# wwyuan2023/VITS

Hardware: AMD Instinct MI355X
Metric: 22.05 kHz audio samples/sec/GPU (infer RTF) + train utt/sec at 1/2/4/8 MI355X (higher is better)
Workload: dtype fp32; 1 GPU; SynthesizerTrn.infer_p2 batch=16 Tx=100 Ty=500 (configs/base.json, 16 kHz, hop 192) per GPU; global_batch=16, seq_len=500, parallelism=single GPU, graph=False

## Files before the change

### include/vits_amd.h

```cpp
#ifndef VITS_AMD_H
#define VITS_AMD_H

#include <stdint.h>

#ifdef __cplusplus
extern "C" {
#endif

#define VITS_OK 0
#define VITS_E_ARG (-1)
#define VITS_E_SHAPE (-2)
#define VITS_E_UNSUP (-3)


#define VITS_EPI_STORE 0
#define VITS_EPI_GATE 1
#define VITS_EPI_UPSAMPLE 2

#define VITS_ACT_NONE 0
#define VITS_ACT_RELU 1
#define VITS_ACT_TANH 2
#define VITS_ACT_EXP 3

#define VITS_TILE_128x128 0
// ... 280 lines not shown
  const float* w1;
  int32_t m_pad1;
  int32_t cin_pad1;
  int32_t kc1;
  int32_t k;
  int32_t dil;
  int32_t kc2;
  const float* b1;
  const float* cond;
  int64_t cond_bstride;
  const float* w2;
  int32_t m_pad2;
  int32_t cin_pad2;
  const float* b2;
  float* y;
  int64_t y_bstride;
  int32_t y_cstride;
  int32_t accumulate;
  float post_div;
  int32_t len_skip;
  const int32_t* lengths;
} vits_resblock_pair_desc;
int vits_resblock_pair_forward(const vits_resblock_pair_desc* d, int n, int batch, void* stream);
int vits_resblock_pair_kc(int channels, int k, int dil, int* kc1, int* kc2);
int vits_resblock_pair16_forward(const vits_resblock_pair_desc* d, int n, int batch, int wdtype,
                                 void* stream);
int vits_resblock_pair16_mean_forward(const vits_resblock_pair_desc* d, int n, int batch,
                                      int wdtype, void* stream);
int vits_resblock_pair_f32p_forward(const vits_resblock_pair_desc* d, int n, int batch,
                                    void* stream);
int vits_resblock_pair_f32p_mean_forward(const vits_resblock_pair_desc* d, int n, int batch,
                                         void* stream);

#define VITS_RADAM_MAX 96
typedef struct vits_radam_tensor {
  float* param;
  const float* grad;
  float* exp_avg;
  float* exp_avg_sq;
  int64_t numel;
} vits_radam_tensor;
int vits_radam_step(const vits_radam_tensor* tensors, int n, float* scal, const float* found_inf,
                    const float* grad_scale, double lr, const double* lr_dev, double beta1,
                    double beta2, double eps, double weight_decay, void* stream);

#define VITS_WNORM_MAX 56
typedef struct vits_wnorm_layer {
  const float* v;
  const float* g;
  float* w;
  const float* dw;
  float* dv;
  float* dg;
  int32_t rows;
  int32_t cols;
} vits_wnorm_layer;
int vits_weight_norm_forward(const vits_wnorm_layer* layers, int n, float* norms, void* stream);
int vits_weight_norm_backward(const vits_wnorm_layer* layers, int n, const float* norms,
                              void* stream);

#define VITS_SNORM_MAX 48
typedef struct vits_snorm_layer {
  const float* w;
  float* u;
  float* v;
  float* w_sn;
// ... 100 lines not shown
```

### vits_amd/_lib.py

```python
from __future__ import annotations

import ctypes as C
import os
import threading

_LIB_PATH = os.path.join(os.path.dirname(os.path.abspath(__file__)), "lib", "libvits_amd.so")
_LIB_PATH = os.environ.get("VITS_AMD_LIB", _LIB_PATH)
_lock = threading.Lock()
_lib = None

VITS_OK = 0
VITS_E_ARG = -1
VITS_E_SHAPE = -2
VITS_E_UNSUP = -3

EPI_STORE, EPI_GATE, EPI_UPSAMPLE = 0, 1, 2
ACT_NONE, ACT_RELU, ACT_TANH, ACT_EXP = 0, 1, 2, 3
TILE_128x128, TILE_64x256, TILE_32x256, TILE_64x128 = 0, 1, 2, 3
WDT_F32, WDT_BF16, WDT_F16, WDT_F32S, WDT_F32P = 0, 1, 2, 3, 4
TILE_ROWS = {TILE_128x128: 128, TILE_64x256: 64, TILE_32x256: 32, TILE_64x128: 64}
DT_F32, DT_F16, DT_BF16, DT_I32 = 0, 1, 2, 3


class ConvOut(C.Structure):
# ... 53 lines not shown

class ResblockPairDesc(C.Structure):
    _fields_ = [
        ("x", C.c_void_p),
        ("x_bstride", C.c_int64),
        ("x_cstride", C.c_int32),
        ("t_len", C.c_int32),
        ("channels", C.c_int32),
        ("in_slope", C.c_float),
        ("w1", C.c_void_p),
        ("m_pad1", C.c_int32),
        ("cin_pad1", C.c_int32),
        ("kc1", C.c_int32),
        ("k", C.c_int32),
        ("dil", C.c_int32),
        ("kc2", C.c_int32),
        ("b1", C.c_void_p),
        ("cond", C.c_void_p),
        ("cond_bstride", C.c_int64),
        ("w2", C.c_void_p),
        ("m_pad2", C.c_int32),
        ("cin_pad2", C.c_int32),
        ("b2", C.c_void_p),
        ("y", C.c_void_p),
        ("y_bstride", C.c_int64),
        ("y_cstride", C.c_int32),
        ("accumulate", C.c_int32),
        ("post_div", C.c_float),
        ("len_skip", C.c_int32),
        ("lengths", C.c_void_p),
    ]


class StftJob(C.Structure):
    _fields_ = [
        ("x", C.c_void_p),
        ("window", C.c_void_p),
        ("grad_mag", C.c_void_p),
        ("mag", C.c_void_p),
        ("re", C.c_void_p),
        ("im", C.c_void_p),
        ("grad_x", C.c_void_p),
        ("batch", C.c_int32),
        ("length", C.c_int32),
        ("n_fft", C.c_int32),
        ("hop", C.c_int32),
        ("win", C.c_int32),
        ("pad", C.c_int32),
        ("eps", C.c_float),
        ("layout", C.c_int32),
    ]


class ConvWgradDesc(C.Structure):
    _fields_ = [
        ("dy", C.c_void_p),
        ("dy_bstride", C.c_int64),
        ("dy_cstride", C.c_int32),
        ("cout", C.c_int32),
        ("x", C.c_void_p),
        ("x_bstride", C.c_int64),
        ("x_cstride", C.c_int32),
        ("cin", C.c_int32),
        ("tin", C.c_int32),
        ("n_out", C.c_int32),
        ("k", C.c_int32),
# ... 194 lines not shown
        C.c_int, [C.c_void_p, C.c_void_p, C.c_int, C.c_int, C.c_int, C.c_float, C.c_void_p]),
    "vits_conv1d_pack16": (
        C.c_int,
        [C.c_void_p] + [C.c_int] * 4 + [C.c_void_p] + [C.c_int] * 3
        + [C.c_void_p, C.c_int64, C.c_void_p],
    ),
    "vits_conv1d_pack16_pair": (
        C.c_int,
        [C.c_void_p] + [C.c_int] * 3 + [C.c_void_p] + [C.c_int] * 2 + [C.c_void_p]
        + [C.c_int] * 3 + [C.c_void_p],
    ),
    "vits_conv1d_pack16_pairs": (C.c_int, [C.POINTER(Pack16Layer), C.c_int, C.c_int,
                                           C.c_void_p]),
    "vits_conv1d_wgrad": (C.c_int, [C.POINTER(ConvWgradDesc), C.c_int, C.c_void_p]),
    "vits_conv1d_wgrad_workspace": (C.c_int64, [C.POINTER(ConvWgradDesc), C.c_int]),
    "vits_conv1d_wgrad_split": (C.c_int, [C.POINTER(ConvWgradDesc), C.c_int, C.c_void_p,
                                          C.c_int64, C.c_void_p]),
    "vits_gate_forward": (
        C.c_int,
        [C.c_void_p, C.c_int64, C.c_int32, C.c_void_p, C.c_int64, C.c_void_p, C.c_int64, C.c_int32,
         C.c_int, C.c_int, C.c_int, C.c_void_p],
    ),
    "vits_gate_backward": (
        C.c_int,
        [C.c_void_p, C.c_int64, C.c_int32, C.c_void_p, C.c_int64, C.c_int32, C.c_void_p, C.c_int64,
         C.c_void_p, C.c_int64, C.c_int32, C.c_void_p, C.c_int, C.c_int, C.c_int, C.c_void_p],
    ),
    "vits_resblock_pair_forward": (
        C.c_int, [C.POINTER(ResblockPairDesc), C.c_int, C.c_int, C.c_void_p]),
    "vits_resblock_pair_f32p_forward": (
        C.c_int, [C.POINTER(ResblockPairDesc), C.c_int, C.c_int, C.c_void_p]),
    "vits_resblock_pair_f32p_mean_forward": (
        C.c_int, [C.POINTER(ResblockPairDesc), C.c_int, C.c_int, C.c_void_p]),
    "vits_resblock_pair_kc": (
        C.c_int, [C.c_int, C.c_int, C.c_int, C.POINTER(C.c_int), C.POINTER(C.c_int)]),
    "vits_resblock_pair16_forward": (
        C.c_int, [C.POINTER(ResblockPairDesc), C.c_int, C.c_int, C.c_int, C.c_void_p]),
    "vits_resblock_pair16_mean_forward": (
        C.c_int, [C.POINTER(ResblockPairDesc), C.c_int, C.c_int, C.c_int, C.c_void_p]),
    "vits_gate_forward_io16": (
        C.c_int,
        [C.c_void_p, C.c_int64, C.c_int32, C.c_void_p, C.c_int64, C.c_void_p, C.c_int64, C.c_int32,
         C.c_int, C.c_int, C.c_int, C.c_int, C.c_void_p],
    ),
    "vits_gate_backward_io16": (
        C.c_int,
        [C.c_void_p, C.c_int64, C.c_int32, C.c_void_p, C.c_int64, C.c_int32, C.c_void_p, C.c_int64,
         C.c_void_p, C.c_int64, C.c_int32, C.c_void_p, C.c_int, C.c_int, C.c_int, C.c_int,
         C.c_void_p],
    ),
    "vits_gate_backward_io16_multi": (
        C.c_int, [C.POINTER(GateBwdJob), C.c_int, C.c_int, C.c_int, C.c_int, C.c_void_p]),
    "vits_radam_step": (
        C.c_int,
        [C.POINTER(RadamTensor), C.c_int, C.c_void_p, C.c_void_p, C.c_void_p, C.c_double,
         C.c_void_p] + [C.c_double] * 4 + [C.c_void_p],
    ),
    "vits_weight_norm_forward": (
        C.c_int, [C.POINTER(WnormLayer), C.c_int, C.c_void_p, C.c_void_p]),
    "vits_weight_norm_backward": (
        C.c_int, [C.POINTER(WnormLayer), C.c_int, C.c_void_p, C.c_void_p]),
    "vits_spectral_norm_supported": (C.c_int, [C.c_int, C.c_int]),
    "vits_spectral_norm_forward": (
        C.c_int, [C.POINTER(SnormLayer), C.c_int, C.c_int, C.c_int, C.c_void_p]),
    "vits_spectral_norm_workspace": (C.c_int64, [C.POINTER(SnormLayer), C.c_int]),
    "vits_spectral_norm_backward": (
# ... 125 lines not shown
```

### vits_amd/csrc/conv1d.hip

```cpp
#include <cstdlib>

#include "conv1d_impl.h"

namespace {

int check_desc(const vits_conv1d_desc& d, int batch) {
  VITS_CHECK_ARG(d.x && d.w && d.out0.y);
  VITS_CHECK_ARG(batch > 0 && d.cin > 0 && d.m > 0 && d.k > 0 && d.dil > 0 && d.n_out > 0);
  VITS_CHECK_SHAPE(d.kc >= 2 && (d.kc % 2) == 0 && d.cin_pad % d.kc == 0 && d.cin_pad >= d.cin);
  VITS_CHECK_SHAPE(d.m_pad % 128 == 0 && d.m_pad >= d.m);
  VITS_CHECK_SHAPE(d.tin >= 0 && d.x_tstride >= 1);
  VITS_CHECK_SHAPE(d.x_tstride != 1 || d.x_cstride >= d.tin);
  if (d.epi == VITS_EPI_GATE) VITS_CHECK_SHAPE((d.m % 2) == 0);
  if (d.epi == VITS_EPI_UPSAMPLE)
    VITS_CHECK_SHAPE(d.up_u > 0 && d.up_u <= 64 && d.m < (1 << 14) && d.m % d.up_u == 0 &&
                     d.t_out > 0);
  if (d.epi == VITS_EPI_STORE && d.split < d.m) VITS_CHECK_ARG(d.out1.y != nullptr);
  if ((reinterpret_cast<uintptr_t>(d.w) & 15) != 0) return VITS_E_SHAPE;
  VITS_CHECK_ARG(d.wdtype == VITS_WDT_F32 || d.wdtype == VITS_WDT_BF16 ||
                 d.wdtype == VITS_WDT_F16 || d.wdtype == VITS_WDT_F32S ||
                 d.wdtype == VITS_WDT_F32P);
  if (d.wdtype == VITS_WDT_F32P) VITS_CHECK_SHAPE(d.kc == 16 || d.kc == 32);
  if (d.wdtype != VITS_WDT_F32) VITS_CHECK_SHAPE((d.kc % 16) == 0);
  if (d.gmask) VITS_CHECK_ARG(d.epi == VITS_EPI_STORE && d.split >= d.m);
// ... 44 lines not shown
  }
  if (rc == VITS_OK) vits_count(which);
  return rc;
}

int conv1d_group_or_seq(const vits_conv1d_desc* d, int n, int batch, hipStream_t s) {
  if (n > 1 && n <= vits_conv::VITS_CONV_GROUP) {
    int rc = conv1d_group(d, n, batch, s);
    if (rc != VITS_E_UNSUP) return rc;
  }
  for (int i = 0; i < n; ++i) {
    int rc = conv1d_group(d + i, 1, batch, s);
    if (rc) return rc;
  }
  return VITS_OK;
}

}

extern "C" int vits_conv1d_forward(const vits_conv1d_desc* d, int batch, void* stream) {
  if (!d) return VITS_E_ARG;
  return conv1d_group(d, 1, batch, as_stream(stream));
}

extern "C" int vits_conv1d_forward_seq(const vits_conv1d_desc* d, int n, int batch, void* stream) {
  if (!d || n < 0) return VITS_E_ARG;
  for (int i = 0; i < n; ++i) {
    int rc = conv1d_group(d + i, 1, batch, as_stream(stream));
    if (rc) return rc;
  }
  return VITS_OK;
}

extern "C" int vits_conv1d_forward_groups(const vits_conv1d_desc* d, const int32_t* sizes,
                                          int ngroups, int batch, void* stream) {
  if (!d || !sizes || ngroups < 0) return VITS_E_ARG;
  int off = 0;
  for (int i = 0; i < ngroups; ++i) {
    VITS_CHECK_ARG(sizes[i] >= 1);
    int rc = conv1d_group_or_seq(d + off, sizes[i], batch, as_stream(stream));
    if (rc) return rc;
    off += sizes[i];
  }
  return VITS_OK;
}
```

### vits_amd/engine.py

```python
from __future__ import annotations

import os

import math
from typing import Optional

import torch

from . import ops
from ._lib import ACT_EXP, ACT_NONE, ACT_RELU, EPI_GATE
from .ops import PackedConv, make_desc, make_out, pack_conv, pack_conv_transpose

_PLAN_ATTR = "_vits_amd_plan"


def _param_signature(module: torch.nn.Module):
    ver = 0
    first = None
    n = 0
    for p in module.parameters():
        ver += p._version
        if first is None:
            first = (p.data_ptr(), p.device, p.dtype)
        n += 1
# ... 33 lines not shown


class _CondStack:

    def __init__(self):
        self.w, self.b, self.n = [], [], 0

    def add(self, weight: torch.Tensor, bias: Optional[torch.Tensor]) -> int:
        off = self.n
        self.w.append(_f32(weight))
        self.b.append(_f32(bias) if bias is not None else torch.zeros(
            weight.shape[0], device=weight.device))
        self.n += weight.shape[0]
        return off

    def finish(self):
        if not self.w:
            return None, None
        return torch.cat(self.w, 0).contiguous(), torch.cat(self.b, 0).contiguous()


def _linear_eff(lin: torch.nn.Module):
    return ops.weight_norm_effective(lin), lin.bias


def _conv_eff(conv: torch.nn.Module):
    return ops.weight_norm_effective(conv), conv.bias


_GROUP_BRANCHES = True
_FUSED_PAIRS = True
MEAN_PAIRS16 = True
MEAN_PAIRS_F32P = True
ACT16 = True


class GeneratorPlan:
    def __init__(self, gen):
        self.signature = None
        dev = _device_of(gen)
        self.num_kernels = gen.num_kernels
        w, b = _conv_eff(gen.conv_pre)
        self.conv_pre = pack_conv(w, b)
        self.ups = []
        self.stages = []
        conds = _CondStack()
        for i, up in enumerate(gen.ups):
            w, b = _conv_eff(up)
            self.ups.append(pack_conv_transpose(w, b, up.stride[0], up.padding[0]))
            blocks = []
            for j in range(gen.num_kernels):
                rb = gen.resblocks[i * gen.num_kernels + j]
                pairs = []
                for c1, c2, cs in zip(rb.convs1, rb.convs2, rb.conds):
                    w1, b1 = _conv_eff(c1)
                    w2, b2 = _conv_eff(c2)
                    wc, bc = _linear_eff(cs)
                    p1 = pack_conv(w1, b1, dilation=c1.dilation[0], padding=c1.padding[0],
                                   gate=True)
                    p2 = pack_conv(w2, b2, dilation=c2.dilation[0], padding=c2.padding[0])
                    alt = None
                    if (ops.PACK_PRECISION.wdtype == ops.WDT_F32S and p1.wdtype == ops.WDT_F32
                            and p2.wdtype == ops.WDT_F32):
                        alt = (ops.to_lowp(p1, ops.WDT_F32S, min_rows=0),
                               ops.to_lowp(p2, ops.WDT_F32S, min_rows=0))
                    pairs.append((p1, p2, conds.add(wc, bc), alt))
# ... 106 lines not shown
                    and all(fused[j][p][0].wdtype == ops.WDT_F32P for j in range(nk))):
                ops.resblock_pair_launch(tuple(pair_desc(j, p, xs) for j in range(nk)), B, dev,
                                         ops.WDT_F32P, mean=True)
                continue
            if cj:
                ops.conv1d_launch_seq(grouped(c1_desc(j, p) for j in cj), B, dev)
            for j in range(nk):
                kw = dict(accumulate=j > 0, post_div=float(nk) if j == nk - 1 else 1.0)
                if fused[j][p]:
                    pair_launch([j], p, [xs], **kw)
                else:
                    ops.conv1d_launch_seq([make_desc(blocks[j][p][1], gbuf[j],
                                                     make_out(xs, res=cur[j], **kw),
                                                     lengths=lengths, io16=io16)], B, dev)


class WNPlan:
    def __init__(self, wn, conds: Optional[_CondStack]):
        self.H = wn.hidden_channels
        self.n_layers = wn.n_layers
        self.cond_off = None
        if wn.gin_channels != 0:
            wc, bc = _linear_eff(wn.cond_layer)
            self.cond_off = conds.add(wc, bc)
        self.in_layers = []
        self.res_skip = []
        for i in range(wn.n_layers):
            w, b = _conv_eff(wn.in_layers[i])
            self.in_layers.append(pack_conv(w, b, dilation=wn.in_layers[i].dilation[0],
                                            padding=wn.in_layers[i].padding[0], gate=True))
            w, b = _conv_eff(wn.res_skip_layers[i])
            self.res_skip.append(pack_conv(w, b))

    def descs(self, h: torch.Tensor, skip: torch.Tensor, abuf: torch.Tensor,
              cond: Optional[torch.Tensor], lengths: Optional[torch.Tensor]):
        H = self.H
        out = []
        for i in range(self.n_layers):
            coff = 0 if self.cond_off is None else self.cond_off + 2 * H * i
            out.append(make_desc(self.in_layers[i], h, make_out(abuf),
                                 cond=cond if self.cond_off is not None else None,
                                 cond_offset=coff))
            last = i == self.n_layers - 1
            if not last:
                out.append(make_desc(self.res_skip[i], abuf, make_out(h, res=h),
                                     out1=make_out(skip, accumulate=i > 0), split=H,
                                     lengths=lengths))
            else:
                out.append(make_desc(self.res_skip[i], abuf,
                                     make_out(skip, accumulate=i > 0), lengths=lengths))
        return out


class CouplingFlowPlan:

    def __init__(self, block):
        self.signature = None
        conds = _CondStack()
        self.layers = []
        flipped = False
        for f in block.flows_reversed:
            if f.__class__.__name__ == "Flip":
                flipped = not flipped
                continue
            assert f.mean_only, "only mean-only couplings are on the hot path"
            half = f.half_channels
            wp, bp = _conv_eff(f.pre)
            wq, bq = _conv_eff(f.post)
            if flipped:
                wp = wp.flip(1)
                wq, bq = wq.flip(0), bq.flip(0)
            self.layers.append(dict(
                half=half, flipped=flipped,
                pre=pack_conv(wp, bp), post=pack_conv(wq, bq),
                wn=WNPlan(f.enc, conds)))
        assert not flipped, "odd number of Flip modules"
        self.cond_w, self.cond_b = conds.finish()
        self.H = self.layers[0]["wn"].H if self.layers else 0

    def conds(self, g):
        if self.cond_w is None:
            return None
        return ops.linear_rows(g, self.cond_w, self.cond_b)

# ... 343 lines not shown
```

### vits_amd/ops.py

```python
from __future__ import annotations

import contextlib
import ctypes as C
import math
import threading
from dataclasses import dataclass, field
from fractions import Fraction
from typing import Optional

import numpy as np
import torch

from . import _lib
from ._lib import (ACT_NONE, WDT_BF16, WDT_F16, WDT_F32, WDT_F32P, WDT_F32S, ConvDesc, ConvOut, EPI_GATE, EPI_STORE,
                   ResblockPairDesc,
                   EPI_UPSAMPLE, TILE_128x128, TILE_32x256, TILE_64x128, TILE_64x256, TILE_ROWS,
                   check)



def _stream_ptr(device: torch.device) -> int:
    return torch.cuda.current_stream(device).cuda_stream


def require_device(*tensors: torch.Tensor):
    for t in tensors:
        if t is None:
            continue
        if t.device.type != "cuda":
            raise _lib.VitsAmdError(
                "vits_amd HIP ops need tensors on a ROCm GPU (device 'cuda'); "
                f"got {t.device}. There is no CPU path.")


def _ptr(t: Optional[torch.Tensor]) -> Optional[int]:
    return None if t is None else t.data_ptr()


_WEIGHT_CACHE: dict = {}


def set_weight_cache(cache: dict) -> dict:
    global _WEIGHT_CACHE
    prev, _WEIGHT_CACHE = _WEIGHT_CACHE, cache
    return prev


def cached_weight(module: torch.nn.Module):
# ... 395 lines not shown
        check(lib.vits_conv1d_forward_groups(arr, sizes, 1, batch, stream.cuda_stream),
              "vits_conv1d_forward_groups")
        e.record(stream)
        self.records.append((s, e, sum(conv_flops(d, batch) for d in group)))
        self.peaks.append(MFMA_PEAK_TFLOPS[group[0].wdtype])
        self.shapes.append("conv " + "+".join(
            f"m{d.m}c{d.cin}k{d.k}d{d.dil}T{d.n_out}e{d.epi}t{d.tile}" for d in group))

    def launch_pairs(self, lib, group, batch, device, wdtype=None, mean=False):
        s = torch.cuda.Event(enable_timing=True)
        e = torch.cuda.Event(enable_timing=True)
        stream = torch.cuda.current_stream(device)
        s.record(stream)
        arr = (ResblockPairDesc * len(group))(*group)
        if wdtype is None:
            check(lib.vits_resblock_pair_forward(arr, len(group), batch, stream.cuda_stream),
                  "vits_resblock_pair_forward")
        elif wdtype == WDT_F32P:
            fn = (lib.vits_resblock_pair_f32p_mean_forward if mean
                  else lib.vits_resblock_pair_f32p_forward)
            check(fn(arr, len(group), batch, stream.cuda_stream),
                  "vits_resblock_pair_f32p_forward")
        else:
            fn = lib.vits_resblock_pair16_mean_forward if mean else lib.vits_resblock_pair16_forward
            check(fn(arr, len(group), batch, int(wdtype), stream.cuda_stream),
                  "vits_resblock_pair16_forward")
        e.record(stream)
        self.records.append((s, e, sum(resblock_pair_flops(d, batch) for d in group)))
        self.peaks.append(MFMA_PEAK_TFLOPS[WDT_F32 if wdtype is None else
                                           WDT_F32S if wdtype == WDT_F32P else wdtype])
        self.shapes.append("pair " + "+".join(
            f"C{d.channels}k{d.k}d{d.dil}T{d.t_len}" for d in group))

    def summary(self):
        torch.cuda.synchronize()
        ms = [s.elapsed_time(e) for s, e, _ in self.records]
        fl = [f for _, _, f in self.records]
        min_ms = sum(f / (pk * 1e9) for f, pk in zip(fl, self.peaks))
        return dict(launches=len(ms), total_ms=float(sum(ms)), total_flops=int(sum(fl)),
                    avg_ms=float(sum(ms) / max(1, len(ms))), mfma_bound_ms=float(min_ms),
                    f32s_flops=int(sum(f for f, pk in zip(fl, self.peaks)
                                       if pk == MFMA_PEAK_TFLOPS[WDT_F32S])))

    def per_launch(self):
        torch.cuda.synchronize()
        return [(lab, s.elapsed_time(e), f)
                for lab, (s, e, f) in zip(self.shapes, self.records)]


_RB_KC = {}


RESBLOCK_PAIR_MAX_K = 7


def resblock_pair_supported(c1: PackedConv, c2: PackedConv, T: int) -> bool:
    C = c2.out_channels
    return (c1.wdtype == WDT_F32 and c2.wdtype == WDT_F32 and C in (32, 64)
            and c1.m == C and c1.cin == C and c2.cin == C // 2 and c1.k == c2.k
            and c1.k <= RESBLOCK_PAIR_MAX_K and c2.dil == 1 and T % 4 == 0
            and _resblock_kc(C, c1.k, c1.dil) is not None)


F32P_PAIR_MAX_K = {32: 11, 64: 11, 128: 11, 256: 3}


# ... 89 lines not shown
    if ConvTimer.active is not None:
        return ConvTimer.active.launch_pairs(lib, group, batch, device, wdtype, mean=mean)
    arr = (ResblockPairDesc * len(group))(*group)
    fn = lib.vits_resblock_pair16_mean_forward if mean else lib.vits_resblock_pair16_forward
    check(fn(arr, len(group), batch, int(wdtype), _stream_ptr(device)),
          "vits_resblock_pair16_forward")


def resblock_pair_flops(d: ResblockPairDesc, batch: int) -> int:
    C_, k, T = d.channels, d.k, d.t_len
    return 2 * batch * T * (C_ * C_ * k + (C_ // 2) * C_ * k)


def resblock_pair_launch(descs, batch: int, device: torch.device, wdtype: int = WDT_F32,
                         mean: bool = False):
    group = tuple(descs) if isinstance(descs, (tuple, list)) else (descs,)
    lib = _lib.load()
    if mean and wdtype != WDT_F32P:
        raise NotImplementedError("branch-mean launch: split-fp32 pairs only")
    if ConvTimer.active is not None:
        return ConvTimer.active.launch_pairs(lib, group, batch, device,
                                             wdtype=WDT_F32P if wdtype == WDT_F32P else None,
                                             mean=mean)
    arr = (ResblockPairDesc * len(group))(*group)
    if wdtype == WDT_F32P:
        fn = (lib.vits_resblock_pair_f32p_mean_forward if mean
              else lib.vits_resblock_pair_f32p_forward)
        check(fn(arr, len(group), batch, _stream_ptr(device)), "vits_resblock_pair_f32p_forward")
        return
    check(lib.vits_resblock_pair_forward(arr, len(group), batch, _stream_ptr(device)),
          "vits_resblock_pair_forward")


def conv1d_launch(desc: ConvDesc, batch: int, device: torch.device):
    lib = _lib.load()
    if ConvTimer.active is not None:
        return ConvTimer.active.launch(lib, desc, batch, device)
    check(lib.vits_conv1d_forward(C.byref(desc), batch, _stream_ptr(device)), "vits_conv1d_forward")


def conv1d_launch_seq(descs, batch: int, device: torch.device):
    lib = _lib.load()
    if ConvTimer.active is not None:
        for d in descs:
            ConvTimer.active.launch(lib, d, batch, device)
        return
    flat, sizes = [], []
    for d in descs:
        group = tuple(d) if isinstance(d, (tuple, list)) else (d,)
        flat.extend(group)
        sizes.append(len(group))
    arr = (ConvDesc * len(flat))(*flat)
    sz = (C.c_int32 * len(sizes))(*sizes)
    check(lib.vits_conv1d_forward_groups(arr, sz, len(sizes), batch, _stream_ptr(device)),
          "vits_conv1d_forward_groups")


def conv1d(x: torch.Tensor, layer: PackedConv, *, in_slope: float = 1.0, act: int = ACT_NONE,
           cond: Optional[torch.Tensor] = None, residual: Optional[torch.Tensor] = None,
           res_scale: float = 1.0, lengths: Optional[torch.Tensor] = None,
           out: Optional[torch.Tensor] = None, accumulate: bool = False,
           post_div: float = 1.0, t_out: Optional[int] = None) -> torch.Tensor:
    require_device(x, cond, residual, lengths)
    B, _, T = x.shape
    io16 = x.dtype != torch.float32
    if layer.epi == EPI_UPSAMPLE:
        T_out = T * layer.up_u if t_out is None else t_out
    else:
        T_out = T
    if out is None:
        out = torch.empty(B, layer.out_channels, T_out, device=x.device, dtype=x.dtype)
    o0 = make_out(out, act=act, res=residual, res_scale=res_scale, accumulate=accumulate,
                  post_div=post_div)
    if lengths is not None:
        lengths = lengths.to(device=x.device, dtype=torch.int32).contiguous()
    d = make_desc(layer, x, o0, in_slope=in_slope, cond=cond, lengths=lengths, t_out=T_out,
                  io16=2 if io16 else 0)
    conv1d_launch(d, B, x.device)
# ... 784 lines not shown
```

Baseline: 79.67 million output samples/s.

## Fuse WaveNet layer in-conv, gate and res/skip conv into one f32p kernel

Adds a HIP kernel that runs a whole WN layer in one launch: the dilated in-layer conv on split-bf16 MFMA, the tanh·sigmoid gate kept in LDS, and the 1x1 res/skip conv with residual and skip accumulation in the epilogue. The layer ping-pongs h between two buffers instead of writing gated activations to global memory and reading them back, which removes a global round trip and one launch per layer. The engine switches to this path when shapes match (H=256, f32p weights), and a new combined sequencer lets it sit alongside ordinary conv launches. In exchange the kernel needs a large LDS footprint and a hand-tuned schedule, and final_h has to track which buffer ends up holding h.

Measured after the change: 81.32 million output samples/s, median of 6. +2.1%, better.

```diff
diff --git a/include/vits_amd.h b/include/vits_amd.h
--- a/include/vits_amd.h
+++ b/include/vits_amd.h
@@ -336,6 +336,42 @@
 int vits_resblock_pair_f32p_mean_forward(const vits_resblock_pair_desc* d, int n, int batch,
                                          void* stream);
 
+typedef struct vits_wn_layer_desc {
+  const float* h;
+  int64_t h_bstride;
+  int32_t h_cstride;
+  int32_t t_len;
+  int32_t hidden;
+  int32_t k;
+  int32_t dil;
+  int32_t last;
+  const void* w1;
+  int32_t m_pad1;
+  int32_t cin_pad1;
+  const float* b1;
+  const float* cond;
+  int64_t cond_bstride;
+  const void* w2;
+  int32_t m_pad2;
+  int32_t cin_pad2;
+  const float* b2;
+  float* h_out;
+  int64_t ho_bstride;
+  int32_t ho_cstride;
+  int32_t accumulate;
+  float* skip;
+  int64_t skip_bstride;
+  int32_t skip_cstride;
+  int32_t len_skip;
+  int32_t ng;
+  int32_t reserved;
+  const int32_t* lengths;
+} vits_wn_layer_desc;
+int vits_wn_layers_f32p_forward(const vits_wn_layer_desc* d, int n, int batch, void* stream);
+int vits_conv1d_wn_seq_forward(const vits_conv1d_desc* convs, int nconv,
+                               const vits_wn_layer_desc* wn, int nwn, const int32_t* kinds, int n,
+                               int batch, void* stream);
+
 #define VITS_RADAM_MAX 96
 typedef struct vits_radam_tensor {
   float* param;
diff --git a/vits_amd/_lib.py b/vits_amd/_lib.py
--- a/vits_amd/_lib.py
+++ b/vits_amd/_lib.py
@@ -109,6 +109,40 @@
     ]
 
 
+class WnLayerDesc(C.Structure):
+    _fields_ = [
+        ("h", C.c_void_p),
+        ("h_bstride", C.c_int64),
+        ("h_cstride", C.c_int32),
+        ("t_len", C.c_int32),
+        ("hidden", C.c_int32),
+        ("k", C.c_int32),
+        ("dil", C.c_int32),
+        ("last", C.c_int32),
+        ("w1", C.c_void_p),
+        ("m_pad1", C.c_int32),
+        ("cin_pad1", C.c_int32),
+        ("b1", C.c_void_p),
+        ("cond", C.c_void_p),
+        ("cond_bstride", C.c_int64),
+        ("w2", C.c_void_p),
+        ("m_pad2", C.c_int32),
+        ("cin_pad2", C.c_int32),
+        ("b2", C.c_void_p),
+        ("h_out", C.c_void_p),
+        ("ho_bstride", C.c_int64),
+        ("ho_cstride", C.c_int32),
+        ("accumulate", C.c_int32),
+        ("skip", C.c_void_p),
+        ("skip_bstride", C.c_int64),
+        ("skip_cstride", C.c_int32),
+        ("len_skip", C.c_int32),
+        ("ng", C.c_int32),
+        ("reserved", C.c_int32),
+        ("lengths", C.c_void_p),
+    ]
+
+
 class StftJob(C.Structure):
     _fields_ = [
         ("x", C.c_void_p),
@@ -369,6 +403,11 @@
         C.c_int, [C.POINTER(ResblockPairDesc), C.c_int, C.c_int, C.c_void_p]),
     "vits_resblock_pair_f32p_mean_forward": (
         C.c_int, [C.POINTER(ResblockPairDesc), C.c_int, C.c_int, C.c_void_p]),
+    "vits_wn_layers_f32p_forward": (
+        C.c_int, [C.POINTER(WnLayerDesc), C.c_int, C.c_int, C.c_void_p]),
+    "vits_conv1d_wn_seq_forward": (
+        C.c_int, [C.POINTER(ConvDesc), C.c_int, C.POINTER(WnLayerDesc), C.c_int,
+                  C.POINTER(C.c_int32), C.c_int, C.c_int, C.c_void_p]),
     "vits_resblock_pair_kc": (
         C.c_int, [C.c_int, C.c_int, C.c_int, C.POINTER(C.c_int), C.POINTER(C.c_int)]),
     "vits_resblock_pair16_forward": (
diff --git a/vits_amd/csrc/conv1d.hip b/vits_amd/csrc/conv1d.hip
--- a/vits_amd/csrc/conv1d.hip
+++ b/vits_amd/csrc/conv1d.hip
@@ -100,6 +100,30 @@
   return VITS_OK;
 }
 
+int vits_wn_layer_check(const vits_wn_layer_desc& d, int batch);
+int vits_wn_layer_launch(const vits_wn_layer_desc& d, int batch, hipStream_t s);
+
+extern "C" int vits_conv1d_wn_seq_forward(const vits_conv1d_desc* convs, int nconv,
+                                          const vits_wn_layer_desc* wn, int nwn,
+                                          const int32_t* kinds, int n, int batch, void* stream) {
+  if (!kinds || n < 1 || nconv < 0 || nwn < 0 || nconv + nwn != n) return VITS_E_ARG;
+  if ((nconv > 0 && !convs) || (nwn > 0 && !wn)) return VITS_E_ARG;
+  int ic = 0, iw = 0;
+  for (int i = 0; i < n; ++i) {
+    VITS_CHECK_ARG(kinds[i] == 0 || kinds[i] == 1);
+    VITS_CHECK_ARG(kinds[i] ? iw < nwn : ic < nconv);
+    const int rc = kinds[i] ? vits_wn_layer_check(wn[iw++], batch) : check_desc(convs[ic++], batch);
+    if (rc) return rc;
+  }
+  ic = iw = 0;
+  for (int i = 0; i < n; ++i) {
+    const int rc = kinds[i] ? vits_wn_layer_launch(wn[iw++], batch, as_stream(stream))
+                            : conv1d_group(convs + ic++, 1, batch, as_stream(stream));
+    if (rc) return rc;
+  }
+  return VITS_OK;
+}
+
 extern "C" int vits_conv1d_forward_groups(const vits_conv1d_desc* d, const int32_t* sizes,
                                           int ngroups, int batch, void* stream) {
   if (!d || !sizes || ngroups < 0) return VITS_E_ARG;
diff --git a/vits_amd/csrc/wn_f32p.hip b/vits_amd/csrc/wn_f32p.hip
--- /dev/null
+++ b/vits_amd/csrc/wn_f32p.hip
@@ -0,0 +1,427 @@
+#include <type_traits>
+
+#include "conv1d_impl.h"
+
+namespace {
+
+using vits_conv::fast_sigmoid;
+using vits_conv::fast_tanh;
+using vits_conv::split3_bf16x4;
+
+typedef __bf16 bf16x8 __attribute__((ext_vector_type(8)));
+typedef __bf16 bf16x4 __attribute__((ext_vector_type(4)));
+typedef __bf16 bf16x2 __attribute__((ext_vector_type(2)));
+typedef float f32x4v __attribute__((ext_vector_type(4)));
+typedef float f32x2v __attribute__((ext_vector_type(2)));
+
+struct WnArgs {
+  vits_wn_layer_desc d;
+  int batch;
+};
+
+constexpr int WN_KC = 64;
+
+__host__ __device__ inline int wn_xcols(int NG, int k, int dil) {
+  return ((NG + (k - 1) * dil + 3 + 3) >> 2) << 2;
+}
+__host__ __device__ inline int wn_lds_bytes(int H, int NG, int k, int dil) {
+  const int xs = 2 * 3 * wn_xcols(NG, k, dil) * (WN_KC + 4);
+  const int gsz = 3 * NG * (H + 8);
+  return 4 * 4 * H + 2 * (xs > gsz ? xs : gsz) + 64;
+}
+
+__device__ __forceinline__ float wn_gate(float a, float b) {
+#pragma clang fp contract(off)
+  return fast_tanh(a) * fast_sigmoid(b);
+}
+
+template <typename T>
+__device__ __forceinline__ T wn_fresh(T v) {
+  asm volatile("" : "+v"(v));
+  return v;
+}
+
+template <typename T>
+__device__ __forceinline__ const T* wn_sbase(const T* p) {
+  uint64_t u = reinterpret_cast<uint64_t>(p);
+  asm("" : "+s"(u));
+  return (const T*)reinterpret_cast<const __attribute__((address_space(1))) T*>(u);
+}
+
+template <int H, int NG>
+__global__ __launch_bounds__(H * 4, 4) void wn_layer_f32p_kernel(const WnArgs A) {
+  typedef std::integral_constant<bool, true> edge_t;
+  typedef std::integral_constant<bool, false> interior_t;
+  constexpr int M1 = 2 * H;
+  constexpr int NT = (M1 / 32) * 64;
+  constexpr int TN = NG / 32;
+  constexpr int KC = WN_KC;
+  constexpr int KCP = KC + 4;
+  constexpr int GP = H + 8;
+  constexpr int GPL = NG * GP;
+  constexpr int S1 = H / 16, S2 = H / 16;
+  static_assert(NT == H * 4 && NT <= 1024, "threads");
+  static_assert(KC / 4 == NT / 64, "staging: one channel quad per wave");
+  static_assert(NG == 32 || NG == 64, "tile columns");
+  typedef bf16x8 av_t;
+
+  const vits_wn_layer_desc& p = A.d;
+  const int b = blockIdx.z;
+  const int Tn = p.t_len;
+  const int L = p.lengths ? min(Tn, (int)p.lengths[b]) : Tn;
+  const int n0 = blockIdx.x * NG;
+  if (n0 >= Tn) return;
+  if (p.lengths && p.len_skip > 0 && n0 >= L + p.len_skip) return;
+  const int M2 = p.last ? H : 2 * H;
+
+  extern __shared__ float smem[];
+  float* const erow = smem;
+  __bf16* const reg = reinterpret_cast<__bf16*>(smem + 4 * H);
+
+  const int tid = threadIdx.x;
+  const int lane = tid & 63;
+  const int wid = __builtin_amdgcn_readfirstlane(tid >> 6);
+  const int wm = wid * 32;
+  const int l32 = lane & 31;
+  const int lhi = lane >> 5;
+
+  const int k = p.k;
+  const int dil = p.dil;
+  const int p1 = (k - 1) * dil / 2;
+  const int tw0 = n0 - p1;
+  const int xstart = tw0 & ~1;
+  const int xcols = wn_xcols(NG, k, dil);
+  const bool interior = n0 + NG <= L;
+
+  {
+    const float* cond = p.cond ? p.cond + (int64_t)b * p.cond_bstride : nullptr;
+    for (int r = tid; r < 4 * H; r += NT) {
+      float e = 0.f;
+      if (r < M1) {
+        const int idx = (r & 1) ? H + (r >> 1) : (r >> 1);
+        if (p.b1) e = p.b1[idx];
+        if (cond) e += cond[idx];
+      } else if (p.b2 && r - M1 < M2) {
+        e = p.b2[r - M1];
+      }
+      erow[r] = e;
+    }
+  }
+
+  f32x16 acc[TN];
+#pragma unroll
+  for (int j = 0; j < TN; ++j)
+#pragma unroll
+    for (int r = 0; r < 16; ++r) acc[j][r] = 0.f;
+
+  auto mma = [&](const av_t* a, const av_t* bh, const av_t* bm, const av_t* bl) {
+#pragma unroll
+    for (int ni = 0; ni < TN; ++ni) {
+      f32x16 c = acc[ni];
+      c = __builtin_amdgcn_mfma_f32_32x32x16_bf16(a[0], bl[ni], c, 0, 0, 0);
+      c = __builtin_amdgcn_mfma_f32_32x32x16_bf16(a[2], bh[ni], c, 0, 0, 0);
+      c = __builtin_amdgcn_mfma_f32_32x32x16_bf16(a[1], bm[ni], c, 0, 0, 0);
+      c = __builtin_amdgcn_mfma_f32_32x32x16_bf16(a[0], bm[ni], c, 0, 0, 0);
+      c = __builtin_amdgcn_mfma_f32_32x32x16_bf16(a[1], bh[ni], c, 0, 0, 0);
+      c = __builtin_amdgcn_mfma_f32_32x32x16_bf16(a[0], bh[ni], c, 0, 0, 0);
+      acc[ni] = c;
+    }
+  };
+  auto loadA = [&](const __bf16* w, uint32_t al, int64_t wstep, int m_pad, int s, int total,
+                   av_t* a) {
+    const __bf16* wp = w + (int64_t)(s < total ? s : total - 1) * wstep + (int64_t)wm * 8;
+    const uint32_t av = wn_fresh(al);
+#pragma unroll
+    for (int q = 0; q < 3; ++q)
+      a[q] = *reinterpret_cast<const av_t*>(
+          reinterpret_cast<const char*>(wn_sbase(wp + (int64_t)q * m_pad * 8)) + av);
+  };
+
+  constexpr int PF = TN == 1 ? 4 : 2;
+  static_assert((KC / 16) % PF == 0 && S2 % PF == 0, "ring alignment");
+  av_t ar[PF][3];
+  av_t bh[2][TN], bm[2][TN], bl[2][TN];
+
+  const float* xb = p.h + (int64_t)b * p.h_bstride;
+  {
+    const int xsh = tw0 - xstart;
+    const int nblk = xcols >> 1;
+    const int xpl = xcols * KCP;
+    __bf16* const xbuf0 = reg;
+    __bf16* const xbuf1 = reg + 3 * xpl;
+    const int tt = xstart + 2 * lane;
+    const bool xact = lane < nblk;
+    const bool xok = xact && tt >= 0 && tt < Tn;
+    const uint32_t xoff = xok ? (uint32_t)tt * 4u : 0u;
+    f32x2v xr[4];
+    auto gload = [&](int ch) __attribute__((always_inline)) {
+      const float* base = xb + (int64_t)(ch * KC + 4 * wid) * p.h_cstride;
+      const uint32_t xo = wn_fresh(xoff);
+#pragma unroll
+      for (int i = 0; i < 4; ++i) {
+        const float* row = wn_sbase(base + (int64_t)i * p.h_cstride);
+        xr[i] = *reinterpret_cast<const f32x2v*>(reinterpret_cast<const char*>(row) + xo);
+      }
+    };
+    auto lstore = [&](__bf16* xs) __attribute__((always_inline)) {
+      const int fl = wn_fresh(lane);
+      if (fl < nblk) {
+        __bf16* xh = xs + 2 * fl * KCP + 4 * wid;
+#pragma unroll
+        for (int e = 0; e < 2; ++e) {
+          f32x4v w;
+#pragma unroll
+          for (int i = 0; i < 4; ++i) w[i] = xok ? xr[i][e] : 0.f;
+          bf16x4 h4, m4, l4;
+          split3_bf16x4(w, h4, m4, l4);
+          *reinterpret_cast<bf16x4*>(xh + e * KCP) = h4;
+          *reinterpret_cast<bf16x4*>(xh + xpl + e * KCP) = m4;
+          *reinterpret_cast<bf16x4*>(xh + 2 * xpl + e * KCP) = l4;
+        }
+      }
+    };
+    auto loadB = [&](const __bf16* xs, int j, int g, av_t* bh, av_t* bm, av_t* bl) {
+      const int P4 = xpl / 4;
+#pragma unroll
+      for (int ni = 0; ni < TN; ++ni) {
+        const bf16x4* xp = reinterpret_cast<const bf16x4*>(
+            xs + (ni * 32 + l32 + j * dil + xsh) * KCP + 16 * g + 8 * lhi);
+        bh[ni] = __builtin_shufflevector(xp[0], xp[1], 0, 1, 2, 3, 4, 5, 6, 7);
+        bm[ni] = __builtin_shufflevector(xp[P4], xp[P4 + 1], 0, 1, 2, 3, 4, 5, 6, 7);
+        bl[ni] = __builtin_shufflevector(xp[2 * P4], xp[2 * P4 + 1], 0, 1, 2, 3, 4, 5, 6, 7);
+      }
+    };
+    const __bf16* wl = reinterpret_cast<const __bf16*>(p.w1);
+    const uint32_t al = (uint32_t)((lhi * 3) * p.m_pad1 + l32) * 16u;
+    const int64_t wstep = (int64_t)16 * 3 * p.m_pad1;
+    const int total = S1 * k;
+    const int nst = (KC / 16) * k;
+#pragma unroll
+    for (int i = 0; i < PF - 1; ++i) loadA(wl, al, wstep, p.m_pad1, i, total, ar[i]);
+    gload(0);
+    lstore(xbuf0);
+    __syncthreads();
+    for (int ch = 0; ch < H / KC; ++ch) {
+      const bool more = ch + 1 < H / KC;
+      if (more) gload(ch + 1);
+      const __bf16* xs = (ch & 1) ? xbuf1 : xbuf0;
+      const int s0 = ch * nst;
+      int j = 0, g = 0;
+      auto next = [&]() {
+        if (++j == k) {
+          j = 0;
+          ++g;
+        }
+      };
+      loadB(xs, 0, 0, bh[0], bm[0], bl[0]);
+      for (int st = 0; st < nst; st += PF) {
+#pragma unroll
+        for (int u = 0; u < PF; ++u) {
+          loadA(wl, al, wstep, p.m_pad1, s0 + st + u + PF - 1, total, ar[(u + PF - 1) % PF]);
+          next();
+          if (st + u + 1 < nst) loadB(xs, j, g, bh[(u + 1) & 1], bm[(u + 1) & 1], bl[(u + 1) & 1]);
+          __builtin_amdgcn_sched_barrier(0);
+          mma(ar[u], bh[u & 1], bm[u & 1], bl[u & 1]);
+          __builtin_amdgcn_sched_barrier(0);
+        }
+      }
+      if (more) lstore((ch & 1) ? xbuf0 : xbuf1);
+      __syncthreads();
+    }
+  }
+
+  __bf16* const gs = reg;
+  {
+    const int fl = wn_fresh(lane);
+    const int l32 = fl & 31, lhi = fl >> 5;
+    f32x4v er[4];
+#pragma unroll
+    for (int g = 0; g < 4; ++g)
+      er[g] = *reinterpret_cast<const f32x4v*>(erow + wm + 4 * lhi + 8 * g);
+#pragma unroll
+    for (int ni = 0; ni < TN; ++ni) {
+      const int col = ni * 32 + l32;
+#pragma unroll
+      for (int r = 0; r < 16; r += 4) {
+        const int row = wm + 4 * lhi + 8 * (r >> 2);
+        const f32x4v e = er[r >> 2];
+        const float g0 = wn_gate(acc[ni][r] + e[0], acc[ni][r + 1] + e[1]);
+        const float g1 = wn_gate(acc[ni][r + 2] + e[2], acc[ni][r + 3] + e[3]);
+        __bf16* gp = gs + col * GP + (row >> 1);
+        const f32x4v w = {g0, g1, 0.f, 0.f};
+        bf16x4 h4, m4, l4;
+        split3_bf16x4(w, h4, m4, l4);
+        *reinterpret_cast<bf16x2*>(gp) = __builtin_shufflevector(h4, h4, 0, 1);
+        *reinterpret_cast<bf16x2*>(gp + GPL) = __builtin_shufflevector(m4, m4, 0, 1);
+        *reinterpret_cast<bf16x2*>(gp + 2 * GPL) = __builtin_shufflevector(l4, l4, 0, 1);
+      }
+#pragma unroll
+      for (int r = 0; r < 16; ++r) acc[ni][r] = 0.f;
+    }
+  }
+  __syncthreads();
+  if (wm >= M2) return;
+
+  {
+    const int fl = wn_fresh(lane);
+    const int l32 = fl & 31, lhi = fl >> 5;
+    const __bf16* wl = reinterpret_cast<const __bf16*>(p.w2);
+    const uint32_t al = (uint32_t)((lhi * 3) * p.m_pad2 + l32) * 16u;
+    const int64_t wstep = (int64_t)16 * 3 * p.m_pad2;
+    const int total = S2;
+    const __bf16* gl = gs + l32 * GP + 8 * lhi;
+    int g = 0;
+    auto loadB = [&](av_t* bh, av_t* bm, av_t* bl) {
+      const __bf16* x = gl + 16 * g;
+#pragma unroll
+      for (int ni = 0; ni < TN; ++ni) {
+        bh[ni] = *reinterpret_cast<const av_t*>(x + ni * 32 * GP);
+        bm[ni] = *reinterpret_cast<const av_t*>(x + ni * 32 * GP + GPL);
+        bl[ni] = *reinterpret_cast<const av_t*>(x + ni * 32 * GP + 2 * GPL);
+      }
+      ++g;
+    };
+#pragma unroll
+    for (int i = 0; i < PF - 1; ++i) loadA(wl, al, wstep, p.m_pad2, i, total, ar[i]);
+    loadB(bh[0], bm[0], bl[0]);
+    for (int s = 0; s < total; s += PF) {
+#pragma unroll
+      for (int u = 0; u < PF; ++u) {
+        loadA(wl, al, wstep, p.m_pad2, s + u + PF - 1, total, ar[(u + PF - 1) % PF]);
+        if (s + u + 1 < total) loadB(bh[(u + 1) & 1], bm[(u + 1) & 1], bl[(u + 1) & 1]);
+        __builtin_amdgcn_sched_barrier(0);
+        mma(ar[u], bh[u & 1], bm[u & 1], bl[u & 1]);
+        __builtin_amdgcn_sched_barrier(0);
+      }
+    }
+  }
+
+  const bool to_h = !p.last && wm < H;
+  const int yr = (p.last || wm < H) ? wm : wm - H;
+  const float* const rrow = xb + (int64_t)wm * p.h_cstride;
+  float* const yb = to_h ? p.h_out + (int64_t)b * p.ho_bstride + (int64_t)yr * p.ho_cstride
+                         : p.skip + (int64_t)b * p.skip_bstride + (int64_t)yr * p.skip_cstride;
+  const int ycs = to_h ? p.ho_cstride : p.skip_cstride;
+  const bool accum = !to_h && p.accumulate;
+  auto epilogue = [&](auto edge) __attribute__((always_inline)) {
+    const int fl = wn_fresh(lane);
+    const int l32 = fl & 31, lhi = fl >> 5;
+    f32x4v e2[4];
+#pragma unroll
+    for (int g = 0; g < 4; ++g)
+      e2[g] = *reinterpret_cast<const f32x4v*>(erow + M1 + wm + 4 * lhi + 8 * g);
+#pragma unroll
+    for (int ni = 0; ni < TN; ++ni) {
+      const int t = n0 + ni * 32 + l32;
+      const bool st = decltype(edge)::value ? t < Tn : true;
+      const int tc = st ? t : 0;
+      const uint32_t xv = (uint32_t)(4 * lhi * p.h_cstride + tc) * 4u;
+      const uint32_t yv = (uint32_t)(4 * lhi * ycs + tc) * 4u;
+      auto xat = [&](int r) __attribute__((always_inline)) -> const float& {
+        const float* row = rrow + (int64_t)((r & 3) + 8 * (r >> 2)) * p.h_cstride;
+        return *reinterpret_cast<const float*>(reinterpret_cast<const char*>(row) + xv);
+      };
+      auto yat = [&](int r) __attribute__((always_inline)) -> float& {
+        float* row = yb + (int64_t)((r & 3) + 8 * (r >> 2)) * ycs;
+        return *reinterpret_cast<float*>(reinterpret_cast<char*>(row) + yv);
+      };
+      float o[16];
+#pragma unroll
+      for (int r = 0; r < 16; ++r) o[r] = acc[ni][r] + e2[r >> 2][r & 3];
+      if (to_h) {
+        float rv[16];
+#pragma unroll
+        for (int r = 0; r < 16; ++r) rv[r] = xat(r);
+#pragma unroll
+        for (int r = 0; r < 16; ++r) o[r] = rv[r] + o[r];
+      }
+      if (accum) {
+        float yo[16];
+#pragma unroll
+        for (int r = 0; r < 16; ++r) yo[r] = yat(r);
+#pragma unroll
+        for (int r = 0; r < 16; ++r) o[r] = yo[r] + o[r];
+      }
+      if (st) {
+#pragma unroll
+        for (int r = 0; r < 16; ++r) {
+          if constexpr (decltype(edge)::value) o[r] = t < L ? o[r] : 0.f;
+          yat(r) = o[r];
+        }
+      }
+    }
+  };
+  if (interior)
+    epilogue(interior_t());
+  else
+    epilogue(edge_t());
+}
+
+int wn_pick_ng(const vits_wn_layer_desc& d, int batch) {
+  if (d.ng == 32 || d.ng == 64) return d.ng;
+  const long tiles64 = (long)((d.t_len + 63) / 64) * batch;
+  return tiles64 >= 256 ? 64 : 32;
+}
+
+template <int H, int NG>
+int wn_launch(const vits_wn_layer_desc& d, int batch, hipStream_t s) {
+  const int lds = wn_lds_bytes(H, NG, d.k, d.dil);
+  if (lds > 160 * 1024) return VITS_E_UNSUP;
+  WnArgs a;
+  a.d = d;
+  a.batch = batch;
+  hipLaunchKernelGGL((wn_layer_f32p_kernel<H, NG>), dim3((d.t_len + NG - 1) / NG, 1, batch),
+                     dim3(H * 4), lds, s, a);
+  return vits_launch_status();
+}
+
+}
+
+int vits_wn_layer_check(const vits_wn_layer_desc& d, int batch) {
+  VITS_CHECK_ARG(batch >= 1 && batch <= 65535);
+  VITS_CHECK_ARG(d.h && d.w1 && d.w2 && d.skip);
+  VITS_CHECK_ARG(d.last ? d.h_out == nullptr : d.h_out != nullptr);
+  VITS_CHECK_ARG(reinterpret_cast<const void*>(d.h_out) != reinterpret_cast<const void*>(d.h) &&
+                 reinterpret_cast<const void*>(d.skip) != reinterpret_cast<const void*>(d.h) &&
+                 reinterpret_cast<const void*>(d.skip) != reinterpret_cast<const void*>(d.h_out));
+  VITS_CHECK_ARG(d.ng == 0 || d.ng == 32 || d.ng == 64);
+  VITS_CHECK_SHAPE(d.hidden == 256);
+  VITS_CHECK_SHAPE(d.k >= 1 && d.k <= 15 && (d.k & 1) == 1 && d.dil >= 1 && d.t_len > 0);
+  VITS_CHECK_SHAPE((d.k - 1) * d.dil <= 56);
+  const int m2 = d.last ? d.hidden : 2 * d.hidden;
+  VITS_CHECK_SHAPE(d.m_pad1 >= 2 * d.hidden && d.m_pad2 >= m2 && (d.m_pad1 & 3) == 0 &&
+                   (d.m_pad2 & 3) == 0);
+  VITS_CHECK_SHAPE(d.cin_pad1 == d.hidden && d.cin_pad2 == d.hidden);
+  VITS_CHECK_SHAPE((d.t_len & 3) == 0 && (d.h_cstride & 3) == 0 && (d.h_bstride & 3) == 0 &&
+                   d.h_cstride >= d.t_len && d.skip_cstride >= d.t_len &&
+                   (d.last || d.ho_cstride >= d.t_len) &&
+                   (reinterpret_cast<uintptr_t>(d.h) & 15) == 0);
+  VITS_CHECK_SHAPE((reinterpret_cast<uintptr_t>(d.skip) & 3) == 0 &&
+                   (reinterpret_cast<uintptr_t>(d.h_out) & 3) == 0);
+  VITS_CHECK_SHAPE((int64_t)d.hidden * d.h_cstride < (1LL << 31) &&
+                   (int64_t)d.hidden * d.skip_cstride < (1LL << 31) &&
+                   (d.last || (int64_t)d.hidden * d.ho_cstride < (1LL << 31)));
+  VITS_CHECK_SHAPE((reinterpret_cast<uintptr_t>(d.w1) & 15) == 0 &&
+                   (reinterpret_cast<uintptr_t>(d.w2) & 15) == 0);
+  return VITS_OK;
+}
+
+int vits_wn_layer_launch(const vits_wn_layer_desc& d, int batch, hipStream_t s) {
+  const int rc = wn_pick_ng(d, batch) == 64 ? wn_launch<256, 64>(d, batch, s)
+                                            : wn_launch<256, 32>(d, batch, s);
+  return count_ok(rc, VITS_CNT_CONV_SPLIT);
+}
+
+extern "C" int vits_wn_layers_f32p_forward(const vits_wn_layer_desc* d, int n, int batch,
+                                           void* stream) {
+  if (!d || n < 1) return VITS_E_ARG;
+  for (int i = 0; i < n; ++i) {
+    const int rc = vits_wn_layer_check(d[i], batch);
+    if (rc) return rc;
+  }
+  for (int i = 0; i < n; ++i) {
+    const int rc = vits_wn_layer_launch(d[i], batch, as_stream(stream));
+    if (rc) return rc;
+  }
+  return VITS_OK;
+}
diff --git a/vits_amd/engine.py b/vits_amd/engine.py
--- a/vits_amd/engine.py
+++ b/vits_amd/engine.py
@@ -89,6 +89,7 @@
 _FUSED_PAIRS = True
 MEAN_PAIRS16 = True
 MEAN_PAIRS_F32P = True
+_FUSED_WN = True
 ACT16 = True
 
 
@@ -261,10 +262,26 @@
             w, b = _conv_eff(wn.res_skip_layers[i])
             self.res_skip.append(pack_conv(w, b))
 
+    def fused(self, h: torch.Tensor) -> bool:
+        return _FUSED_WN and all(ops.wn_layer_f32p_supported(a, r, h)
+                                 for a, r in zip(self.in_layers, self.res_skip))
+
     def descs(self, h: torch.Tensor, skip: torch.Tensor, abuf: torch.Tensor,
               cond: Optional[torch.Tensor], lengths: Optional[torch.Tensor]):
         H = self.H
         out = []
+        if self.fused(h):
+            cur, nxt = h, abuf
+            for i in range(self.n_layers):
+                coff = 0 if self.cond_off is None else self.cond_off + 2 * H * i
+                last = i == self.n_layers - 1
+                out.append(ops.wn_layer_desc(
+                    self.in_layers[i], self.res_skip[i], cur, None if last else nxt, skip,
+                    accumulate=i > 0, cond=cond if self.cond_off is not None else None,
+                    cond_offset=coff, lengths=lengths))
+                if not last:
+                    cur, nxt = nxt, cur
+            return out
         for i in range(self.n_layers):
             coff = 0 if self.cond_off is None else self.cond_off + 2 * H * i
             out.append(make_desc(self.in_layers[i], h, make_out(abuf),
@@ -279,6 +296,9 @@
                 out.append(make_desc(self.res_skip[i], abuf,
                                      make_out(skip, accumulate=i > 0), lengths=lengths))
         return out
+
+    def final_h(self, h: torch.Tensor, abuf: torch.Tensor) -> torch.Tensor:
+        return abuf if self.fused(h) and self.n_layers % 2 == 0 else h
 
 
 class CouplingFlowPlan:
diff --git a/vits_amd/ops.py b/vits_amd/ops.py
--- a/vits_amd/ops.py
+++ b/vits_amd/ops.py
@@ -13,7 +13,7 @@
 
 from . import _lib
 from ._lib import (ACT_NONE, WDT_BF16, WDT_F16, WDT_F32, WDT_F32P, WDT_F32S, ConvDesc, ConvOut, EPI_GATE, EPI_STORE,
-                   ResblockPairDesc,
+                   ResblockPairDesc, WnLayerDesc,
                    EPI_UPSAMPLE, TILE_128x128, TILE_32x256, TILE_64x128, TILE_64x256, TILE_ROWS,
                    check)
 
@@ -475,6 +475,19 @@
         self.shapes.append("pair " + "+".join(
             f"C{d.channels}k{d.k}d{d.dil}T{d.t_len}" for d in group))
 
+    def launch_wn(self, lib, desc, batch, device):
+        s = torch.cuda.Event(enable_timing=True)
+        e = torch.cuda.Event(enable_timing=True)
+        stream = torch.cuda.current_stream(device)
+        s.record(stream)
+        check(lib.vits_wn_layers_f32p_forward(C.byref(desc), 1, batch, stream.cuda_stream),
+              "vits_wn_layers_f32p_forward")
+        e.record(stream)
+        self.records.append((s, e, wn_layer_flops(desc, batch)))
+        self.peaks.append(MFMA_PEAK_TFLOPS[WDT_F32S])
+        self.shapes.append(f"wn H{desc.hidden}k{desc.k}d{desc.dil}T{desc.t_len}"
+                           + ("last" if desc.last else ""))
+
     def summary(self):
         torch.cuda.synchronize()
         ms = [s.elapsed_time(e) for s, e, _ in self.records]
@@ -630,6 +643,56 @@
           "vits_resblock_pair_forward")
 
 
+WN_NG = 0
+
+
+def wn_layer_f32p_supported(in_layer: PackedConv, res_skip: PackedConv, h: torch.Tensor) -> bool:
+    H = in_layer.cin
+    return (in_layer.wdtype == WDT_F32P and res_skip.wdtype == WDT_F32P and H == 256
+            and h.dtype == torch.float32 and h.dim() == 3 and h.shape[1] == H
+            and in_layer.m == 2 * H and in_layer.epi == EPI_GATE and in_layer.cin_pad == H
+            and in_layer.k % 2 == 1 and (in_layer.k - 1) * in_layer.dil <= 56
+            and in_layer.pad_left == (in_layer.k - 1) * in_layer.dil // 2
+            and res_skip.epi == EPI_STORE and res_skip.k == 1 and res_skip.cin == H
+            and res_skip.cin_pad == H and res_skip.m in (H, 2 * H) and res_skip.pad_left == 0
+            and h.shape[2] % 4 == 0 and h.stride(2) == 1 and h.stride(1) % 4 == 0
+            and h.stride(0) % 4 == 0 and h.data_ptr() % 16 == 0
+            and H * h.stride(1) < 2 ** 31)
+
+
+def wn_layer_desc(in_layer: PackedConv, res_skip: PackedConv, h: torch.Tensor,
+                  h_out: Optional[torch.Tensor], skip: torch.Tensor, *, accumulate: bool,
+                  cond: Optional[torch.Tensor] = None, cond_offset: int = 0,
+                  lengths: Optional[torch.Tensor] = None) -> WnLayerDesc:
+    H, T = h.shape[1], h.shape[2]
+    last = h_out is None
+    assert res_skip.m == (H if last else 2 * H)
+    assert skip.dtype == torch.float32 and skip.stride(2) == 1
+    d = WnLayerDesc()
+    d.h, d.h_bstride, d.h_cstride, d.t_len = h.data_ptr(), h.stride(0), h.stride(1), T
+    d.hidden, d.k, d.dil, d.last = H, in_layer.k, in_layer.dil, int(last)
+    d.w1, d.m_pad1, d.cin_pad1 = in_layer.w.data_ptr(), in_layer.m_pad, in_layer.cin_pad
+    d.b1 = _ptr(in_layer.bias)
+    if cond is not None:
+        d.cond, d.cond_bstride = cond.data_ptr() + 4 * cond_offset, cond.stride(0)
+    d.w2, d.m_pad2, d.cin_pad2 = res_skip.w.data_ptr(), res_skip.m_pad, res_skip.cin_pad
+    d.b2 = _ptr(res_skip.bias)
+    if not last:
+        assert h_out.dtype == torch.float32 and h_out.stride(2) == 1
+        d.h_out, d.ho_bstride, d.ho_cstride = h_out.data_ptr(), h_out.stride(0), h_out.stride(1)
+    d.skip, d.skip_bstride, d.skip_cstride = skip.data_ptr(), skip.stride(0), skip.stride(1)
+    d.accumulate = int(accumulate)
+    d.lengths = _ptr(lengths)
+    d.len_skip = LEN_SKIP.margin if lengths is not None else 0
+    d.ng = WN_NG
+    return d
+
+
+def wn_layer_flops(d: WnLayerDesc, batch: int) -> int:
+    H = d.hidden
+    return 2 * batch * d.t_len * (2 * H * H * d.k + (H if d.last else 2 * H) * H)
+
+
 def conv1d_launch(desc: ConvDesc, batch: int, device: torch.device):
     lib = _lib.load()
     if ConvTimer.active is not None:
@@ -641,7 +704,20 @@
     lib = _lib.load()
     if ConvTimer.active is not None:
         for d in descs:
-            ConvTimer.active.launch(lib, d, batch, device)
+            if isinstance(d, WnLayerDesc):
+                ConvTimer.active.launch_wn(lib, d, batch, device)
+            else:
+                ConvTimer.active.launch(lib, d, batch, device)
+        return
+    if any(isinstance(d, WnLayerDesc) for d in descs):
+        convs = [d for d in descs if not isinstance(d, WnLayerDesc)]
+        wns = [d for d in descs if isinstance(d, WnLayerDesc)]
+        assert all(isinstance(d, ConvDesc) for d in convs), "no grouped launches beside WN layers"
+        kinds = (C.c_int32 * len(descs))(*[int(isinstance(d, WnLayerDesc)) for d in descs])
+        check(lib.vits_conv1d_wn_seq_forward((ConvDesc * len(convs))(*convs), len(convs),
+                                             (WnLayerDesc * len(wns))(*wns), len(wns), kinds,
+                                             len(descs), batch, _stream_ptr(device)),
+              "vits_conv1d_wn_seq_forward")
         return
     flat, sizes = [], []
     for d in descs:
```
